# j042/mimi

Measured on AMD Instinct MI355X. Metric: element-integrations/sec (residual+Jacobian assembly), higher is better.
Workload: dtype f64

## Files before the change

mimi_amd/csrc/kernels_tensor_wgs.hpp:

```cpp
#pragma once

#include <hip/hip_runtime.h>

#include "materials_other.hpp"

#include "kernels_tensor_2phase.hpp"

namespace mimi_hip {

struct P2Shape {
  static constexpr int P = 2, NB = 3, NQ = 4, NB2 = 9, ND = 27, NQ3 = 64, NROW = 81;
};

constexpr int p2_stage_r_size(int rows) {
  using S = P2Shape;
  return rows * 3 * (S::NQ3 + S::NB * S::NQ * S::NQ + S::NB2 * S::NQ);
}

struct WgsLds : P2Shape {
  static constexpr int off_tab = 0;
  static constexpr int off_r = off_tab + 2 * 6 * NB * NQ;
  static constexpr int off_ah = off_r + p2_stage_r_size(1);
  static constexpr int n_final = 9 * NROW + 18 * ND;
  static constexpr int n_carry = 18 * 2 * ND;
  static constexpr int st_size = n_final + 1;
  static constexpr int off_st = off_ah + 3 * ND * NQ3;
  static constexpr int total = off_st + 3 * st_size;
};

#define WGS_PIN(x) asm volatile("" : "+v"(x))

MH_DEV void wgs_barrier() {
  asm volatile("s_waitcnt lgkmcnt(0)\n\ts_barrier" ::: "memory");
}

MH_DEV void swap32_f64(double c, double o, double& c_hi_in_lo, double& o_lo_in_hi) {
  const unsigned long long uc = __double_as_longlong(c), uo = __double_as_longlong(o);
  const auto lo = __builtin_amdgcn_permlane32_swap((unsigned)uc, (unsigned)uo, false, false);
  const auto hi = __builtin_amdgcn_permlane32_swap((unsigned)(uc >> 32), (unsigned)(uo >> 32), false, false);
  o_lo_in_hi = __longlong_as_double(((unsigned long long)hi[0] << 32) | lo[0]);
  c_hi_in_lo = __longlong_as_double(((unsigned long long)hi[1] << 32) | lo[1]);
}

constexpr int WGS_PT_FIELDS = 24;

MH_DEV void wgs_point_store(double* rec, int lane, const mimi_hip_material& m, const PointResult<3>& w) {
  constexpr int NQ3 = P2Shape::NQ3;
  constexpr int sym_i[6] = {0, 1, 2, 1, 2, 2}, sym_j[6] = {0, 0, 0, 1, 1, 2};
#pragma unroll
  for (int k = 0; k < 9; ++k) rec[k * NQ3 + lane] = w.Finv[k];
  rec[9 * NQ3 + lane] = w.detF;
#pragma unroll
  for (int k = 0; k < 6; ++k) {
    rec[(10 + k) * NQ3 + lane] = w.sigma[sym_i[k] + 3 * sym_j[k]];
    rec[(16 + k) * NQ3 + lane] = w.s_trial[sym_i[k] + 3 * sym_j[k]];
  }
  double beta, gamma;
  j2_beta_gamma<3>(m, w, beta, gamma);
  rec[22 * NQ3 + lane] = beta;
  rec[23 * NQ3 + lane] = gamma;
}

MH_DEV void wgs_point_load(const double* rec, int lane, PointResult<3>& w, double& beta, double& gamma) {
  constexpr int NQ3 = P2Shape::NQ3;
  constexpr int sym_i[6] = {0, 1, 2, 1, 2, 2}, sym_j[6] = {0, 0, 0, 1, 1, 2};
#pragma unroll
  for (int k = 0; k < 9; ++k) w.Finv[k] = rec[k * NQ3 + lane];
  w.detF = rec[9 * NQ3 + lane];
#pragma unroll
  for (int k = 0; k < 6; ++k) {
    const double sg = rec[(10 + k) * NQ3 + lane], st = rec[(16 + k) * NQ3 + lane];
    w.sigma[sym_i[k] + 3 * sym_j[k]] = sg;
    w.sigma[sym_j[k] + 3 * sym_i[k]] = sg;
    w.s_trial[sym_i[k] + 3 * sym_j[k]] = st;
    w.s_trial[sym_j[k] + 3 * sym_i[k]] = st;
  }
  beta = rec[22 * NQ3 + lane];
  gamma = rec[23 * NQ3 + lane];
  pk1_from_cauchy<3>(w);
}

constexpr int WGS_REC_FIELDS = 90;
constexpr int WGS_KIND_RECORD = 100;

template<int FAMILY, int COMMIT = 0>
__global__ __launch_bounds__(256) void tensor_point_kernel(TensorArgs p, int n_el) {
  constexpr int P = P2Shape::P, NB = P2Shape::NB, NQ = P2Shape::NQ, ND = P2Shape::ND, NQ3 = P2Shape::NQ3;
  constexpr int FK = family_kind<FAMILY>();
  __shared__ double ue_all[4][3 * ND];
  __shared__ double tab_all[4][6 * NB * NQ];
  const int wave = threadIdx.x >> 6, lane = threadIdx.x & 63;
  const int64_t e = (int64_t)blockIdx.x * 4 + wave;
  if (e >= n_el) return;
  double* ue = ue_all[wave];
  double* tab = tab_all[wave];
  int el[3];
  el[0] = e % p.box_n[0];
  el[1] = (e / p.box_n[0]) % p.box_n[1];
  el[2] = e / ((int64_t)p.box_n[0] * p.box_n[1]);
  const int32_t* dofs = p.dofs + e * ND;
  for (int a = lane; a < ND; a += 64) {
    const int64_t node = dofs[a];
    for (int c = 0; c < 3; ++c) ue[c * ND + a] = p.u[node * 3 + c];
  }
  for (int t = lane; t < 6 * NB * NQ; t += 64) {
    const int dir = t / (2 * NB * NQ), rem = t % (2 * NB * NQ), isD = rem / (NB * NQ), k = rem % (NB * NQ);
    const int span = p.box_begin[dir] + el[dir];
    tab[t] = ((isD ? p.tabD[dir] : p.tabB[dir]) + (int64_t)span * NB * NQ)[k];
  }
  __builtin_amdgcn_s_waitcnt(0);
  __builtin_amdgcn_wave_barrier();
  const int q0 = lane % NQ, q1 = (lane / NQ) % NQ, q2 = lane / (NQ * NQ);
  double H[9];
  for (int k = 0; k < 9; ++k) H[k] = 0.0;
#pragma unroll 1
  for (int a2 = 0; a2 < NB; ++a2)
#pragma unroll 1
    for (int a1 = 0; a1 < NB; ++a1)
      for (int a0 = 0; a0 < NB; ++a0) {
        const int a = a0 + NB * (a1 + NB * a2);
        const double b0 = tab_ptr<P>(tab, 0, 0)[a0 * NQ + q0], d0 = tab_ptr<P>(tab, 0, 1)[a0 * NQ + q0];
        const double b1 = tab_ptr<P>(tab, 1, 0)[a1 * NQ + q1], d1 = tab_ptr<P>(tab, 1, 1)[a1 * NQ + q1];
        const double b2 = tab_ptr<P>(tab, 2, 0)[a2 * NQ + q2], d2 = tab_ptr<P>(tab, 2, 1)[a2 * NQ + q2];
        const double dn0 = d0 * (b1 * b2), dn1 = b0 * (d1 * b2), dn2 = b0 * (b1 * d2);
        for (int i = 0; i < 3; ++i) {
          const double uu = ue[i * ND + a];
          H[i * 3 + 0] += uu * dn0;
          H[i * 3 + 1] += uu * dn1;
          H[i * 3 + 2] += uu * dn2;
        }
      }
  const double* g = p.geo + e * 10 * NQ3 + lane;
  double F[9];
  for (int i = 0; i < 3; ++i)
    for (int J = 0; J < 3; ++J) {
      double sf = (i == J) ? 1.0 : 0.0;
      for (int m = 0; m < 3; ++m) sf += H[i * 3 + m] * g[(int64_t)(m * 3 + J) * NQ3];
      F[i + J * 3] = sf;
    }
  if constexpr (COMMIT) {
    int st;
    if constexpr (FAMILY != 0) st = accumulate_other<3, FK>(p.mat, p.dt, p.state, e * NQ3 + lane, F);
    else st = accumulate_state<3>(p.mat, p.dt, p.state, e * NQ3 + lane, F);
    if (st) atomicOr(p.status, st);
    return;
  }
  if constexpr (FAMILY != 0) {
    double Pk[9];
    OtherTangent<3> ot;
    const int status = other_tangent_begin<3, FK>(p.mat, p.dt, p.state, e * NQ3 + lane, F, Pk, ot);
    double* rec = p.scratch_pt + e * (int64_t)(WGS_REC_FIELDS * NQ3) + lane;
    const double wd = g[(int64_t)9 * NQ3];
    double Ji[9];
#pragma unroll
    for (int k = 0; k < 9; ++k) Ji[k] = g[(int64_t)k * NQ3];
#pragma unroll 1
    for (int j = 0; j < 3; ++j) {
      double acc[27];
#pragma unroll
      for (int k = 0; k < 27; ++k) acc[k] = 0.0;
#pragma unroll 1
      for (int L = 0; L < 3; ++L) {
        double dP[9];
        other_tangent_dir<3, FK>(p.mat, p.dt, F, ot, j, L, dP);
        double jl[3];
#pragma unroll
        for (int n = 0; n < 3; ++n) jl[n] = L == 0 ? Ji[n * 3] : (L == 1 ? Ji[n * 3 + 1] : Ji[n * 3 + 2]);
#pragma unroll
        for (int i = 0; i < 3; ++i)
#pragma unroll
          for (int m = 0; m < 3; ++m) {
            double b = 0.0;
#pragma unroll
            for (int J = 0; J < 3; ++J) b += Ji[m * 3 + J] * dP[i + J * 3];
#pragma unroll
            for (int n = 0; n < 3; ++n) acc[(i * 3 + m) * 3 + n] += b * jl[n];
          }
      }
#pragma unroll
      for (int i = 0; i < 3; ++i)
#pragma unroll
        for (int m = 0; m < 3; ++m)
#pragma unroll
          for (int n = 0; n < 3; ++n) rec[(int64_t)(i * 27 + (m * 3 + j) * 3 + n) * NQ3] = wd * acc[(i * 3 + m) * 3 + n];
    }
#pragma unroll
    for (int i = 0; i < 3; ++i)
#pragma unroll
      for (int m = 0; m < 3; ++m) {
        double t = 0.0;
#pragma unroll
        for (int J = 0; J < 3; ++J) t += Pk[i + J * 3] * Ji[m * 3 + J];
        rec[(int64_t)(81 + i * 3 + m) * NQ3] = wd * t;
      }
    if (status) atomicOr(p.status, status);
  } else {
    PointResult<3> w;
    const int status = evaluate_pk1<3>(p.mat, p.dt, p.state, e * NQ3 + lane, F, w);
    wgs_point_store(p.scratch_pt + e * (int64_t)(WGS_PT_FIELDS * NQ3), lane, p.mat.m, w);
    if (status) atomicOr(p.status, status);
  }
}

template<int KIND>
struct WgsPoint;

template<>
struct WgsPoint<MIMI_HIP_MAT_NEOHOOKEAN> {
  double G[9], M[6], Phat[9];
  double mu_w, c1_w, c2_w;
};

template<>
struct WgsPoint<MIMI_HIP_MAT_J2> {
  double G[9], Ji[9], N[9], Q[9], sig[9], st[9], Phat[9];
  double wdJ, Kc, hb, gg;
};

template<>
struct WgsPoint<WGS_KIND_RECORD> {
  const double* rec;
};

MH_DEV void wgs_j2_point(const mimi_hip_material& m, const PointResult<3>& w, double beta, double gamma, const double* Ji,
                         double wd, WgsPoint<MIMI_HIP_MAT_J2>& s) {
  const double G2 = 2.0 * m.G;
  s.wdJ = wd * w.detF;
  s.Kc = m.K - beta * G2 / 3.0;
  s.hb = 0.5 * beta * G2;
  s.gg = G2 * gamma;
#pragma unroll
  for (int k = 0; k < 9; ++k) {
    s.Ji[k] = Ji[k];
    s.sig[k] = w.sigma[k];
    s.st[k] = w.s_trial[k];
  }
#pragma unroll
  for (int mm = 0; mm < 3; ++mm)
#pragma unroll
    for (int c = 0; c < 3; ++c) {
      double g = 0.0;
#pragma unroll
      for (int Jx = 0; Jx < 3; ++Jx) g += Ji[mm * 3 + Jx] * w.Finv[Jx + c * 3];
      s.G[mm * 3 + c] = g;
    }
#pragma unroll
  for (int mm = 0; mm < 3; ++mm)
#pragma unroll
    for (int n = 0; n < 3; ++n) {
      double v = 0.0;
#pragma unroll
      for (int k = 0; k < 3; ++k) v += s.G[mm * 3 + k] * Ji[n * 3 + k];
      s.N[mm * 3 + n] = v;
    }
#pragma unroll
  for (int n = 0; n < 3; ++n)
#pragma unroll
    for (int j = 0; j < 3; ++j) {
      double v = 0.0;
#pragma unroll
      for (int Lx = 0; Lx < 3; ++Lx) v += w.s_trial[j + Lx * 3] * Ji[n * 3 + Lx];
      s.Q[n * 3 + j] = v;
    }
#pragma unroll
  for (int i = 0; i < 3; ++i)
#pragma unroll
    for (int mm = 0; mm < 3; ++mm) {
      double sp = 0.0;
#pragma unroll
      for (int Jx = 0; Jx < 3; ++Jx) sp += w.P[i + Jx * 3] * Ji[mm * 3 + Jx];
      s.Phat[i * 3 + mm] = wd * sp;
    }
}

MH_DEV void wgs_neohookean_point(const mimi_hip_material& mat, const double* F, const double* Ji, double wd,
                                 WgsPoint<MIMI_HIP_MAT_NEOHOOKEAN>& s) {
  PointResult<3> w;
  neo_hookean_stress<3>(mat, F, w);
  const double J = w.detF;
  s.mu_w = wd * mat.mu;
  s.c1_w = wd * (mat.lambda * J * (J - 1.) - mat.mu);
  s.c2_w = wd * (mat.lambda * (2. * J - 1.) * J);
#pragma unroll
  for (int m = 0; m < 3; ++m)
#pragma unroll
    for (int i = 0; i < 3; ++i) {
      double g = 0.0;
#pragma unroll
      for (int Jx = 0; Jx < 3; ++Jx) g += Ji[m * 3 + Jx] * w.Finv[Jx + i * 3];
      s.G[m * 3 + i] = g;
    }
  {
    int c = 0;
#pragma unroll
    for (int m = 0; m < 3; ++m)
#pragma unroll
      for (int n = m; n < 3; ++n) {
        double v = 0.0;
#pragma unroll
        for (int Jx = 0; Jx < 3; ++Jx) v += Ji[m * 3 + Jx] * Ji[n * 3 + Jx];
        s.M[c++] = v;
      }
  }
#pragma unroll
  for (int i = 0; i < 3; ++i)
#pragma unroll
    for (int m = 0; m < 3; ++m) {
      double sp = 0.0;
#pragma unroll
      for (int Jx = 0; Jx < 3; ++Jx) sp += w.P[i + Jx * 3] * Ji[m * 3 + Jx];
      s.Phat[i * 3 + m] = wd * sp;
    }
}

template<int ROWS>
MH_DEV void p2_stage_r(const double* tab, double* RS, int lane, double* er, int I0) {
  using S = P2Shape;
  constexpr int P = S::P, NB = S::NB, NQ = S::NQ, NB2 = S::NB2, ND = S::ND, NQ3 = S::NQ3;
  double* PH = RS;
  double* V = PH + ROWS * 3 * NQ3;
  double* W = V + ROWS * 3 * NB * NQ * NQ;
  __builtin_amdgcn_wave_barrier();
  if (lane < NB * NQ * NQ) {
    const int q01 = lane & 15, a2 = lane >> 4;
    double T[2][NQ];
#pragma unroll
    for (int v = 0; v < 2; ++v)
#pragma unroll
      for (int q2 = 0; q2 < NQ; ++q2) T[v][q2] = tab_ptr<P>(tab, 2, v)[a2 * NQ + q2];
#pragma unroll
    for (int im = 0; im < ROWS * 3; ++im) {
      double sv = 0.0;
#pragma unroll
      for (int q2 = 0; q2 < NQ; ++q2) sv = __builtin_fma(T[im % 3 == 2 ? 1 : 0][q2], PH[im * NQ3 + q01 + NQ * NQ * q2], sv);
      V[im * (NB * NQ * NQ) + lane] = sv;
    }
  }
  __builtin_amdgcn_wave_barrier();
  if (lane < NB2 * NQ) {
    const int q0 = lane & 3, a12 = lane >> 2, a1 = a12 % NB, a2 = a12 / NB;
    double T[2][NQ];
#pragma unroll
    for (int v = 0; v < 2; ++v)
#pragma unroll
      for (int q1 = 0; q1 < NQ; ++q1) T[v][q1] = tab_ptr<P>(tab, 1, v)[a1 * NQ + q1];
#pragma unroll
    for (int im = 0; im < ROWS * 3; ++im) {
      double sw = 0.0;
#pragma unroll
      for (int q1 = 0; q1 < NQ; ++q1) sw = __builtin_fma(T[im % 3 == 1 ? 1 : 0][q1], V[(im * NB + a2) * NQ * NQ + q0 + NQ * q1], sw);
      W[im * (NB2 * NQ) + lane] = sw;
    }
  }
  __builtin_amdgcn_wave_barrier();
  if (lane < (ROWS > 1 ? 2 : 1) * ND) {
    const int a = lane < ND ? lane : lane - ND, a0 = a % NB, a12 = a / NB;
    double T[2][NQ];
#pragma unroll
    for (int v = 0; v < 2; ++v)
#pragma unroll
      for (int q0 = 0; q0 < NQ; ++q0) T[v][q0] = tab_ptr<P>(tab, 0, v)[a0 * NQ + q0];
    const int n_rows = lane < ND ? (ROWS + 1) / 2 : ROWS / 2;
    for (int k = 0; k < n_rows; ++k) {
      const int I = lane < ND ? 2 * k : 2 * k + 1;
      double sr = 0.0;
#pragma unroll
      for (int m = 0; m < 3; ++m)
#pragma unroll
        for (int q0 = 0; q0 < NQ; ++q0) sr = __builtin_fma(T[m == 0 ? 1 : 0][q0], W[((I * 3 + m) * NB2 + a12) * NQ + q0], sr);
      er[a * 3 + I0 + I] = sr;
    }
  }
  __builtin_amdgcn_wave_barrier();
}

template<int KIND, int I>
MH_DEV void wgs_x_row(const TensorArgs& p, double* lds, int lane, int64_t e, int par, const WgsPoint<KIND>& s) {
  using L = WgsLds;
  constexpr int NB = L::NB, NQ = L::NQ, ND = L::ND, NQ3 = L::NQ3;
  static_assert(KIND == MIMI_HIP_MAT_J2 || KIND == WGS_KIND_RECORD, "nine-block kernel: the material comes from the pre-pass");
  const double* tab = lds + L::off_tab + par * 6 * NB * NQ;
  double* AH = lds + L::off_ah + I * ND * NQ3;
  double* RS = lds + L::off_r;
  double Phat[3];
  if constexpr (KIND == WGS_KIND_RECORD) {
#pragma unroll
    for (int m = 0; m < 3; ++m) Phat[m] = s.rec[(int64_t)(81 + I * 3 + m) * NQ3];
    double v[ND];
#pragma unroll
    for (int k = 0; k < ND; ++k) v[k] = s.rec[(int64_t)(I * ND + k) * NQ3];
#pragma unroll
    for (int k = 0; k < ND; ++k) AH[k * NQ3 + lane] = v[k];
  } else {
#pragma unroll
    for (int m = 0; m < 3; ++m) Phat[m] = s.Phat[I * 3 + m];
    double S[3], Ts[3];
#pragma unroll
    for (int m = 0; m < 3; ++m) {
      double a = 0.0, b = 0.0;
#pragma unroll
      for (int k = 0; k < 3; ++k) {
        a += s.sig[I + k * 3] * s.G[m * 3 + k];
        b += s.st[I + k * 3] * s.G[m * 3 + k];
      }
      S[m] = a;
      Ts[m] = b;
    }
#pragma unroll
    for (int m = 0; m < 3; ++m)
#pragma unroll
      for (int j = 0; j < 3; ++j)
#pragma unroll
        for (int n = 0; n < 3; ++n) {
          double v = s.G[n * 3 + j] * S[m] - s.G[m * 3 + j] * S[n];
          v += s.Kc * s.G[m * 3 + I] * s.Ji[n * 3 + j];
          v += s.hb * ((I == j ? s.N[m * 3 + n] : 0.0) + s.G[m * 3 + j] * s.Ji[n * 3 + I]);
          v -= s.gg * Ts[m] * s.Q[n * 3 + j];
          AH[((m * 3 + j) * 3 + n) * NQ3 + lane] = s.wdJ * v;
        }
  }
#pragma unroll
  for (int m = 0; m < 3; ++m) RS[m * NQ3 + lane] = Phat[m];
  p2_stage_r<1>(tab, RS, lane, p.scratch_r + e * ND * 3, I);
}

struct ColumnWalk {
  int first, nseg;
  int g, pos, unit;
  int cx, cy, ez;
  int64_t e;
  MH_DEV ColumnWalk(const TensorArgs& p, int first_unit) : first(first_unit), nseg(p.box_n[2] / p.seg_len), g(0) { begin_unit(p, 0); }
  MH_DEV void begin_unit(const TensorArgs& p, int u) {
    const int un = first + u, col = un / nseg;
    unit = u;
    pos = 0;
    cx = col % p.box_n[0];
    cy = col / p.box_n[0];
    ez = (un % nseg) * p.seg_len;
    e = cx + (int64_t)p.box_n[0] * (cy + (int64_t)p.box_n[1] * ez);
  }
  MH_DEV void advance(const TensorArgs& p) {
    ++g;
    if (++pos == p.seg_len) {
      begin_unit(p, unit + 1);
    } else {
      ++ez;
      e += (int64_t)p.box_n[0] * p.box_n[1];
    }
  }
};

struct WgsOperands {
  static constexpr int NT = 6 * P2Shape::NB * P2Shape::NQ, TROUNDS = 2;
  double tab[TROUNDS], geo[10];
  MH_DEV static const double* table_src(const TensorArgs& p, const ColumnWalk& c, int t) {
    constexpr int NBQ = P2Shape::NB * P2Shape::NQ;
    const int dir = t / (2 * NBQ);
    const int rem = t % (2 * NBQ);
    const int isD = rem / NBQ;
    const int k = rem % NBQ;
    const int span = (dir == 0 ? p.box_begin[0] + c.cx : dir == 1 ? p.box_begin[1] + c.cy : p.box_begin[2] + c.ez);
    return (isD ? (dir == 0 ? p.tabD[0] : dir == 1 ? p.tabD[1] : p.tabD[2])
                : (dir == 0 ? p.tabB[0] : dir == 1 ? p.tabB[1] : p.tabB[2])) + (int64_t)span * NBQ + k;
  }
  MH_DEV void request(const TensorArgs& p, const ColumnWalk& c, int lane) {
#pragma unroll
    for (int rd = 0; rd < TROUNDS; ++rd) {
      const int t = rd * 64 + lane;
      tab[rd] = *table_src(p, c, t < NT ? t : 0);
    }
    const double* g = p.geo + c.e * 10 * P2Shape::NQ3 + lane;
#pragma unroll
    for (int k = 0; k < 10; ++k) geo[k] = g[(int64_t)k * P2Shape::NQ3];
  }
  MH_DEV void tables_to_lds(double* dst, int lane) const {
#pragma unroll
    for (int rd = 0; rd < TROUNDS; ++rd) {
      const int t = rd * 64 + lane;
      if (t < NT) dst[t] = tab[rd];
    }
  }
};

template<int KIND>
MH_DEV void wgs_x_loop(const TensorArgs& p, double* lds, int unit) {
  using L = WgsLds;
  const int lane = threadIdx.x & 63;
  const int n_seq = p.seg_len;
  ColumnWalk cq(p, unit);
  ColumnWalk cs = cq;
  ColumnWalk cr = cq;
  WgsOperands op;
  auto request = [&]() {
    op.request(p, cq, lane);
    if (cq.g + 1 < n_seq) cq.advance(p);
  };
  WgsPoint<KIND> s;
  auto point_stage = [&]() {
    op.tables_to_lds(lds + L::off_tab + (cs.g & 1) * WgsOperands::NT, lane);
    if constexpr (KIND == WGS_KIND_RECORD) {
      s.rec = p.scratch_pt + cs.e * (int64_t)(WGS_REC_FIELDS * L::NQ3) + lane;
    } else {
      PointResult<3> w;
      double beta, gamma;
      wgs_point_load(p.scratch_pt + cs.e * (int64_t)(WGS_PT_FIELDS * L::NQ3), lane, w, beta, gamma);
      wgs_j2_point(p.mat.m, w, beta, gamma, op.geo, op.geo[9], s);
    }
    __builtin_amdgcn_wave_barrier();
    if (cs.g + 1 < n_seq) cs.advance(p);
  };
  auto rows = [&]() {
    wgs_x_row<KIND, 0>(p, lds, lane, cr.e, cr.g & 1, s);
    wgs_x_row<KIND, 1>(p, lds, lane, cr.e, cr.g & 1, s);
    wgs_x_row<KIND, 2>(p, lds, lane, cr.e, cr.g & 1, s);
  };
  request();
  point_stage();
  if (1 < n_seq) request();
  rows();
  wgs_barrier();
  for (int it = 0; it < n_seq; ++it) {
    if (it + 1 < n_seq) {
      point_stage();
      if (it + 2 < n_seq) request();
    }
    wgs_barrier();
    if (it + 1 < n_seq) {
      cr.advance(p);
      rows();
    }
    wgs_barrier();
  }
}

struct WgsLane {
  int lane, grp;
  bool col_ok;
  double take_c0, take_c1;
  int base0, stride0, base1, basec;
  int baseT0, strideT0, baseT1, basecT;
};

MH_DEV WgsLane wgs_lane_constants(bool for_dump = false) {
  constexpr int NB = P2Shape::NB, ND = P2Shape::ND, NROW = P2Shape::NROW;
  WgsLane c;
  c.lane = threadIdx.x & 63;
  const int col = c.lane & 15;
  c.grp = c.lane >> 4;
  c.col_ok = col < 9;
  c.take_c0 = c.grp != 2 ? 1.0 : 0.0;
  c.take_c1 = c.grp == 0 ? 1.0 : 0.0;
  const int a0 = c.col_ok ? col / NB : 0, b0 = c.col_ok ? col % NB : 0;
  const int grp = c.grp;
  c.base0 = grp < 3 ? a0 * NROW + grp * ND + b0 * 3 : 9 * NROW + a0 * ND + b0 * 3;
  c.stride0 = grp < 3 ? 3 * NROW : 3 * ND;
  c.base1 = 9 * NROW + (a0 + 9) * ND + b0 * 3;
  c.basec = a0 * 162 + b0 * 3 + (grp == 0 ? 0 : grp == 1 ? ND : grp == 3 ? 9 * 162 : 9 * 162 + ND);
  c.baseT0 = grp == 0 ? b0 * NROW + a0 * 3
           : grp == 3 ? b0 * NROW + ND + a0 * 3
           : grp == 1 ? 9 * NROW + b0 * ND + a0 * 3
                      : 9 * NROW + (b0 + 9) * ND + a0 * 3;
  c.strideT0 = (grp == 0 || grp == 3) ? 3 * NROW : 3 * ND;
  c.baseT1 = b0 * NROW + 2 * ND + a0 * 3;
  c.basecT = b0 * 162 + a0 * 3 + (grp == 0 ? 0 : grp == 1 ? 9 * 162 : grp == 3 ? ND : 9 * 162 + ND);
  if (for_dump) {
    if (!c.col_ok) c.base0 = c.stride0 = c.baseT0 = c.strideT0 = 0;
    if (!c.col_ok || grp != 2) c.base1 = c.baseT1 = 0;
  }
  return c;
}

template<int MODE, bool DUMP = false>
MH_DEV void wgs_contract_block(const WgsLane& lc, const double (&ah)[9], const double (&aS0)[4], const double (&aS2)[4],
                               const double (&uB1)[3][4], const double (&uD1)[3][4], double (&C)[9],
                               double* st_n, int jn, double* st_t, int jt, double* dump = nullptr) {
  constexpr int NB = P2Shape::NB, NQ = P2Shape::NQ, ND = P2Shape::ND, NROW = P2Shape::NROW;
  const mh_d4 zero4 = {0.0, 0.0, 0.0, 0.0};
  const int grp = lc.grp;
  double* const dn0 = lc.col_ok ? st_n : dump;
  double* const dn1 = (lc.col_ok && grp == 2) ? st_n : dump;
  double* const dt0 = lc.col_ok ? st_t : dump;
  double* const dt1 = (lc.col_ok && grp == 2) ? st_t : dump;
  mh_d4 D1[9];
#pragma unroll
  for (int mn = 0; mn < 9; ++mn) {
    const int m = mn / 3, n = mn % 3;
    const int v2 = (m == 2 ? 1 : 0) + (n == 2 ? 2 : 0);
    if (MODE == 2 && mn == 3) D1[3] = D1[1];
    else D1[mn] = __builtin_amdgcn_mfma_f64_16x16x4f64(ah[mn], aS2[v2], zero4, 0, 0, 0);
  }
  mh_d4 Kt[NB];
  auto carry_and_stage = [&](int b1) {
#pragma unroll
    for (int a1 = 0; a1 < NB; ++a1) {
      if (MODE == 2 && a1 < b1) continue;
      const int a1b1 = a1 * NB + b1;
      const double cin = C[a1b1];
      double c_rot, o2_rot;
      swap32_f64(cin, Kt[a1][2], c_rot, o2_rot);
      const double out0 = MODE == 0 ? Kt[a1][0] + (grp != 2 ? cin : 0.0) : __builtin_fma(cin, lc.take_c0, Kt[a1][0]);
      const double out1 = MODE == 0 ? Kt[a1][1] + (grp == 0 ? c_rot : 0.0) : __builtin_fma(c_rot, lc.take_c1, Kt[a1][1]);
      if constexpr (DUMP) {
        dn0[lc.base0 + a1 * lc.stride0 + b1 * 9 + jn] = out0;
        dn1[lc.base1 + a1 * (3 * ND) + b1 * 9 + jn] = out1;
        if (MODE == 1 || (MODE == 2 && a1 > b1)) {
          dt0[lc.baseT0 + b1 * lc.strideT0 + a1 * 9 + jt] = out0;
          dt1[lc.baseT1 + b1 * (3 * NROW) + a1 * 9 + jt] = out1;
        }
      } else {
        if (lc.col_ok) st_n[lc.base0 + a1 * lc.stride0 + b1 * 9 + jn] = out0;
        if (lc.col_ok && grp == 2) st_n[lc.base1 + a1 * (3 * ND) + b1 * 9 + jn] = out1;
        if (MODE == 1 || (MODE == 2 && a1 > b1)) {
          if (lc.col_ok) st_t[lc.baseT0 + b1 * lc.strideT0 + a1 * 9 + jt] = out0;
          if (lc.col_ok && grp == 2) st_t[lc.baseT1 + b1 * (3 * NROW) + a1 * 9 + jt] = out1;
        }
      }
      C[a1b1] = grp == 2 ? o2_rot : out1;
    }
  };
#pragma unroll
  for (int b1 = 0; b1 < NB; ++b1) {
    double Ec[4][NB];
#pragma unroll
    for (int q1 = 0; q1 < NQ; ++q1) {
      const double cbB = uB1[b1][q1], cbD = uD1[b1][q1];
      const double W3 = cbB * D1[0][q1];
      const double W1 = __builtin_fma(cbD, D1[1][q1], cbB * D1[2][q1]);
      const double W2a = cbB * D1[3][q1], W2b = cbB * D1[6][q1];
      const double W0a = __builtin_fma(cbD, D1[4][q1], cbB * D1[5][q1]);
      const double W0b = __builtin_fma(cbD, D1[7][q1], cbB * D1[8][q1]);
#pragma unroll
      for (int a1 = 0; a1 < NB; ++a1) {
        if (MODE == 2 && a1 < b1) continue;
        const double caB = uB1[a1][q1], caD = uD1[a1][q1];
        if (q1 == 0) {
          Ec[3][a1] = caB * W3;
          Ec[1][a1] = caB * W1;
          Ec[2][a1] = __builtin_fma(caD, W2a, caB * W2b);
          Ec[0][a1] = __builtin_fma(caD, W0a, caB * W0b);
        } else {
          Ec[3][a1] = __builtin_fma(caB, W3, Ec[3][a1]);
          Ec[1][a1] = __builtin_fma(caB, W1, Ec[1][a1]);
          Ec[2][a1] = __builtin_fma(caD, W2a, __builtin_fma(caB, W2b, Ec[2][a1]));
          Ec[0][a1] = __builtin_fma(caD, W0a, __builtin_fma(caB, W0b, Ec[0][a1]));
        }
      }
    }
    if (b1 > 0) carry_and_stage(b1 - 1);
#pragma unroll
    for (int g = 0; g < 4; ++g)
#pragma unroll
      for (int a1 = 0; a1 < NB; ++a1)
        if (!(MODE == 2 && a1 < b1)) WGS_PIN(Ec[g][a1]);
#pragma unroll
    for (int a1 = 0; a1 < NB; ++a1)
      if (!(MODE == 2 && a1 < b1)) Kt[a1] = __builtin_amdgcn_mfma_f64_16x16x4f64(Ec[0][a1], aS0[0], zero4, 0, 0, 0);
#pragma unroll
    for (int g = 1; g < 4; ++g)
#pragma unroll
      for (int a1 = 0; a1 < NB; ++a1)
        if (!(MODE == 2 && a1 < b1)) Kt[a1] = __builtin_amdgcn_mfma_f64_16x16x4f64(Ec[g][a1], aS0[g], Kt[a1], 0, 0, 0);
  }
  carry_and_stage(NB - 1);
}

template<int MODE>
MH_DEV void wgs_stage_carry(const WgsLane& lc, const double (&C)[9], double* st_n, int jn, double* st_t, int jt) {
  constexpr int NB = P2Shape::NB;
#pragma unroll
  for (int a1b1 = 0; a1b1 < 9; ++a1b1) {
    const int a1 = a1b1 / NB, b1 = a1b1 % NB;
    if (MODE == 2 && a1 < b1) continue;
    if (lc.col_ok) st_n[lc.basec + a1 * 486 + b1 * 9 + jn] = C[a1b1];
    if ((MODE == 1 || (MODE == 2 && a1 > b1)) && lc.col_ok) st_t[lc.basecT + b1 * 486 + a1 * 9 + jt] = C[a1b1];
  }
}

#define WGS_PIECE_STORE(ptr, v) (*(ptr) = (v))
MH_DEV void wgs_flush_final(int lane, const double* ST, double* E, int I) {
  constexpr int NROW = P2Shape::NROW, ND = P2Shape::ND;
  {
    const int g3 = lane / 17, k3 = lane - 17 * g3;
    const bool ok3 = lane < 51;
    const int src3 = ok3 ? g3 * NROW + 64 + k3 : 0, dst3 = g3 * 3 * NROW + 64 + k3;
    double v0[9], v1[3];
#pragma unroll
    for (int a = 0; a < 9; ++a) v0[a] = ST[a * NROW + lane];
#pragma unroll
    for (int q = 0; q < 3; ++q) v1[q] = ST[q * 3 * NROW + src3];
    double* d = E + I * NROW;
#pragma unroll
    for (int a = 0; a < 9; ++a) WGS_PIECE_STORE(&d[(unsigned)(a * 3 * NROW + lane)], v0[a]);
#pragma unroll
    for (int q = 0; q < 3; ++q)
      if (ok3) WGS_PIECE_STORE(&d[(unsigned)(q * 9 * NROW + dst3)], v1[q]);
  }
  {
    const int half = lane >> 5, k = lane & 31;
    const bool ok = k < ND;
    double w[9];
#pragma unroll
    for (int r = 0; r < 9; ++r) w[r] = ST[9 * NROW + (2 * r + half) * ND + (ok ? k : 0)];
    double* d = E + P2Block::off_b20 + I * ND + half * NROW + k;
#pragma unroll
    for (int r = 0; r < 9; ++r)
      if (ok) WGS_PIECE_STORE(&d[(unsigned)(2 * r * NROW)], w[r]);
  }
}

MH_DEV void wgs_load_tables(const double* tab, int lane, bool column_too, double (&aS0)[4], double (&aS2)[4],
                            double (&uB1)[P2Shape::NB][P2Shape::NQ], double (&uD1)[P2Shape::NB][P2Shape::NQ]) {
  constexpr int P = P2Shape::P, NB = P2Shape::NB, NQ = P2Shape::NQ;
  const int mrow = lane & 15, mk = lane >> 4;
  const bool mrow_ok = mrow < P2Shape::NB2;
  const int mra = mrow_ok ? mrow / NB : 0, mrb = mrow_ok ? mrow % NB : 0;
  auto pair_products = [&](int dir, double (&aS)[4]) {
    const double Ba = tab_ptr<P>(tab, dir, 0)[mra * NQ + mk], Da = tab_ptr<P>(tab, dir, 1)[mra * NQ + mk];
    const double Bb = tab_ptr<P>(tab, dir, 0)[mrb * NQ + mk], Db = tab_ptr<P>(tab, dir, 1)[mrb * NQ + mk];
    aS[0] = mrow_ok ? Ba * Bb : 0.0;
    aS[1] = mrow_ok ? Da * Bb : 0.0;
    aS[2] = mrow_ok ? Ba * Db : 0.0;
    aS[3] = mrow_ok ? Da * Db : 0.0;
  };
  if (column_too) {
    pair_products(0, aS0);
#pragma unroll
    for (int a = 0; a < NB; ++a)
#pragma unroll
      for (int q1 = 0; q1 < NQ; ++q1) {
        const unsigned long long vb = __double_as_longlong(tab_ptr<P>(tab, 1, 0)[a * NQ + q1]);
        const unsigned long long vd = __double_as_longlong(tab_ptr<P>(tab, 1, 1)[a * NQ + q1]);
        const unsigned blo = __builtin_amdgcn_readfirstlane((unsigned)vb), bhi = __builtin_amdgcn_readfirstlane((unsigned)(vb >> 32));
        const unsigned dlo = __builtin_amdgcn_readfirstlane((unsigned)vd), dhi = __builtin_amdgcn_readfirstlane((unsigned)(vd >> 32));
        uB1[a][q1] = __longlong_as_double(((unsigned long long)bhi << 32) | blo);
        uD1[a][q1] = __longlong_as_double(((unsigned long long)dhi << 32) | dlo);
      }
  }
  pair_products(2, aS2);
}

template<int I>
MH_DEV void wgs_y_loop(const TensorArgs& p, double* lds, int unit) {
  using L = WgsLds;
  constexpr int NB = L::NB, NQ = L::NQ, NB2 = L::NB2, ND = L::ND, NQ3 = L::NQ3;
  const WgsLane lc = wgs_lane_constants();
  const int lane = lc.lane;
  double* AH = lds + L::off_ah + I * ND * NQ3;
  double* ST = lds + L::off_st + I * L::st_size;
  const int n_seq = p.seg_len;
  ColumnWalk c(p, unit);
  auto block_of = [&](int64_t e) -> double* { return p.scratch_k + e * (int64_t)P2Block::size; };

  double C[3][NB2];
#pragma unroll
  for (int j = 0; j < 3; ++j)
#pragma unroll
    for (int k = 0; k < NB2; ++k) C[j][k] = 0.0;
  double aS0[4], aS2[4];
  double uB1[NB][NQ], uD1[NB][NQ];
  auto load_slice = [&](int j, double (&ah)[9]) {
#pragma unroll
    for (int m = 0; m < 3; ++m)
#pragma unroll
      for (int n = 0; n < 3; ++n) ah[m * 3 + n] = AH[((m * 3 + j) * 3 + n) * NQ3 + lane];
  };
  wgs_barrier();
  for (int it = 0; it < n_seq; ++it) {
    wgs_load_tables(lds + L::off_tab + (it & 1) * WgsOperands::NT, lane, true, aS0, aS2, uB1, uD1);
    {
      double ah[9];
      load_slice(0, ah);
      wgs_contract_block<0>(lc, ah, aS0, aS2, uB1, uD1, C[0], ST, 0, ST, 0);
    }
    {
      double ah[9];
      load_slice(1, ah);
      wgs_contract_block<0>(lc, ah, aS0, aS2, uB1, uD1, C[1], ST, 1, ST, 1);
    }
    {
      double ah[9];
      load_slice(2, ah);
      wgs_barrier();
      wgs_contract_block<0>(lc, ah, aS0, aS2, uB1, uD1, C[2], ST, 2, ST, 2);
      __builtin_amdgcn_wave_barrier();
      wgs_flush_final(lane, ST, block_of(c.e), I);
      __builtin_amdgcn_wave_barrier();
      wgs_barrier();
    }
    if (it + 1 < n_seq) c.advance(p);
  }
  {
    double* Sc = P2Block::carry_of(block_of(c.e), I);
#pragma unroll
    for (int jj = 0; jj < 3; ++jj) wgs_stage_carry<0>(lc, C[jj], Sc, jj, Sc, jj);
  }
}

template<int KIND>
__global__ __launch_bounds__(256, 2) void tensor_wgs_kernel(TensorArgs p) {
  extern __shared__ __align__(16) double smem_wgs[];
#ifndef WGS_ROT
#define WGS_ROT(b) ((b) >> 3)
#endif
  const int role = __builtin_amdgcn_readfirstlane((int)((threadIdx.x >> 6) + WGS_ROT(blockIdx.x)) & 3);
  const int unit = blockIdx.x;
  if (role == 0) wgs_x_loop<KIND>(p, smem_wgs, unit);
  else if (role == 1) wgs_y_loop<0>(p, smem_wgs, unit);
  else if (role == 2) wgs_y_loop<1>(p, smem_wgs, unit);
  else wgs_y_loop<2>(p, smem_wgs, unit);
}

inline void launch_tensor_wgs(mimi_hip_domain_s* h, const DomainCall& c, TensorArgs a) {
  h->scratch_k.resize((size_t)h->n_el * P2Block::size);
  h->scratch_r.resize((size_t)h->n_el * 3 * 27);
  a.scratch_k = h->scratch_k.ptr;
  a.scratch_r = h->scratch_r.ptr;
  a.n_units_u = a.box_n[0];
  a.n_units_v = a.box_n[1];
  const size_t lds = WgsLds::total * sizeof(double);
  const int kind = h->mat.m.kind;
  h->scratch_pt.resize((size_t)h->n_el * (material_closed_form(kind) ? WGS_PT_FIELDS : WGS_REC_FIELDS) * 64);
  a.scratch_pt = h->scratch_pt.ptr;
  by_material_family(kind, [&](auto K) {
    constexpr int FK = decltype(K)::value;
    run_two_phase(
        h, c, true,
        [&] { launch(tensor_point_kernel<FK>, dim3((unsigned)((h->n_el + 3) / 4)), dim3(256), 0, h->stream, a, (int)h->n_el); },
        [&] {
          auto kernel = FK != 0 ? tensor_wgs_kernel<WGS_KIND_RECORD> : tensor_wgs_kernel<MIMI_HIP_MAT_J2>;
          launch(kernel, dim3(a.box_n[0] * a.box_n[1]), dim3(256), lds, h->stream, a);
        },
        [&] { launch_tensor_p2(h, a); });
  });
}

inline void launch_tensor_p2_post(mimi_hip_domain_s* h, TensorArgs a) {
  by_material_family(h->mat.m.kind, [&](auto K) {
    launch(tensor_point_kernel<decltype(K)::value, 1>, dim3((unsigned)((h->n_el + 3) / 4)), dim3(256), 0, h->stream, a, (int)h->n_el);
  });
}

}
```

mimi_amd/csrc/kernels_tensor_wgsym.hpp:

```cpp
#pragma once

#include <hip/hip_runtime.h>

#include "kernels_tensor_wgs.hpp"

namespace mimi_hip {

#ifndef WGSYM_SPLIT_BELOW
#define WGSYM_SPLIT_BELOW 512
#endif
#ifndef WGSYM_MAX_COLS
#define WGSYM_MAX_COLS 4
#define WGSYM_MIN_WGS 2048
#endif

#ifndef WGSYM_DIAG_MODE
#define WGSYM_DIAG_MODE 2
#endif

struct WgsymLds : P2Shape {
  static constexpr int off_ue = 0;
  static constexpr int off_tab = off_ue + 3 * ND + 1;
  static constexpr int off_r = off_tab + 2 * 6 * NB * NQ;
  static constexpr int off_ah = off_r + p2_stage_r_size(3);
  static constexpr int off_st = off_ah + 6 * 9 * NQ3;
  static constexpr int off_dump = off_st + 3 * WgsLds::st_size;
  static constexpr int total = off_dump + 512;
  MH_DEV static constexpr int ah_block(int i, int j) { return (i * (i + 1) / 2 + j) * 9; }
};

template<int KIND>
MH_DEV void wgsym_x_rows(const TensorArgs& p, double* lds, int lane, int64_t e, int par, const WgsPoint<KIND>& s) {
  using L = WgsymLds;
  constexpr int ND = L::ND, NQ3 = L::NQ3;
  static_assert(KIND == MIMI_HIP_MAT_NEOHOOKEAN, "symmetric-half kernel: hyperelastic materials only");
  const double* tab = lds + L::off_tab + par * WgsOperands::NT;
  double* AH = lds + L::off_ah;
  double* PH = lds + L::off_r;
#pragma unroll
  for (int I = 0; I < 3; ++I)
#pragma unroll
    for (int m = 0; m < 3; ++m) {
      const double c2gm = s.c2_w * s.G[m * 3 + I];
#pragma unroll
      for (int j = 0; j <= I; ++j) {
        const double c1gm = s.c1_w * s.G[m * 3 + j];
#pragma unroll
        for (int n = 0; n < 3; ++n) {
          double v = c2gm * s.G[n * 3 + j] - c1gm * s.G[n * 3 + I];
          if (I == j) {
            const int lo = m < n ? m : n, hi = m < n ? n : m;
            v += s.mu_w * s.M[lo * 3 - lo * (lo - 1) / 2 + (hi - lo)];
          }
          AH[(L::ah_block(I, j) + m * 3 + n) * NQ3 + lane] = v;
        }
      }
    }
#pragma unroll
  for (int k = 0; k < 9; ++k) PH[k * NQ3 + lane] = s.Phat[k];
  p2_stage_r<3>(tab, PH, lane, p.scratch_r + e * ND * 3, 0);
}

template<int KIND>
MH_DEV void wgsym_x_loop(const TensorArgs& p, double* lds, int col0, int n_cols) {
  using L = WgsymLds;
  constexpr int P = L::P, NB = L::NB, NQ = L::NQ, ND = L::ND;
  const int lane = threadIdx.x & 63;
  double* ue = lds + L::off_ue;
  const int n_seq = n_cols * p.seg_len;
  ColumnWalk cq(p, col0);
  ColumnWalk cs = cq;
  ColumnWalk cr = cq;
  int32_t node_n = lane < ND ? p.dofs[cq.e * ND + lane] : 0;
  double ue_r[3];
  WgsOperands op;
  auto request = [&]() {
#pragma unroll
    for (int c = 0; c < 3; ++c) ue_r[c] = p.u[(int64_t)node_n * 3 + c];
    op.request(p, cq, lane);
    if (cq.g + 1 < n_seq) {
      cq.advance(p);
      node_n = lane < ND ? p.dofs[cq.e * ND + lane] : 0;
    }
  };
  WgsPoint<KIND> s;
  auto point_stage = [&]() {
    double* tab = lds + L::off_tab + (cs.g & 1) * WgsOperands::NT;
    if (lane < ND) {
#pragma unroll
      for (int c = 0; c < 3; ++c) ue[c * ND + lane] = ue_r[c];
    }
    op.tables_to_lds(tab, lane);
    double Ji[9];
#pragma unroll
    for (int k = 0; k < 9; ++k) Ji[k] = op.geo[k];
    const double wd = op.geo[9];
    __builtin_amdgcn_wave_barrier();
    double F[9];
    {
      const int q0 = lane & 3, q1 = (lane >> 2) & 3, q2 = lane >> 4;
      double b0[NB], d0[NB], b1[NB], d1[NB], b2[NB], d2[NB];
#pragma unroll
      for (int a = 0; a < NB; ++a) {
        b0[a] = tab_ptr<P>(tab, 0, 0)[a * NQ + q0];
        d0[a] = tab_ptr<P>(tab, 0, 1)[a * NQ + q0];
        b1[a] = tab_ptr<P>(tab, 1, 0)[a * NQ + q1];
        d1[a] = tab_ptr<P>(tab, 1, 1)[a * NQ + q1];
        b2[a] = tab_ptr<P>(tab, 2, 0)[a * NQ + q2];
        d2[a] = tab_ptr<P>(tab, 2, 1)[a * NQ + q2];
      }
      double H[9];
#pragma unroll
      for (int k = 0; k < 9; ++k) H[k] = 0.0;
#pragma unroll
      for (int a2 = 0; a2 < NB; ++a2)
#pragma unroll
        for (int a1 = 0; a1 < NB; ++a1) {
          const double tbb = b1[a1] * b2[a2], tdb = d1[a1] * b2[a2], tbd = b1[a1] * d2[a2];
#pragma unroll
          for (int a0 = 0; a0 < NB; ++a0) {
            const int a = a0 + NB * (a1 + NB * a2);
            const double dn0 = d0[a0] * tbb, dn1 = b0[a0] * tdb, dn2 = b0[a0] * tbd;
#pragma unroll
            for (int i = 0; i < 3; ++i) {
              const double uu = ue[i * ND + a];
              H[i * 3 + 0] += uu * dn0;
              H[i * 3 + 1] += uu * dn1;
              H[i * 3 + 2] += uu * dn2;
            }
          }
          #pragma unroll
          for (int k = 0; k < 9; ++k) asm volatile("" : "+v"(H[k]) : : "memory");
        }
#pragma unroll
      for (int i = 0; i < 3; ++i)
#pragma unroll
        for (int J = 0; J < 3; ++J) {
          double sf = (i == J) ? 1.0 : 0.0;
#pragma unroll
          for (int m = 0; m < 3; ++m) sf += H[i * 3 + m] * Ji[m * 3 + J];
          F[i + J * 3] = sf;
        }
    }
    wgs_neohookean_point(p.mat.m, F, Ji, wd, s);
    __builtin_amdgcn_wave_barrier();
    if (cs.g + 1 < n_seq) cs.advance(p);
  };

  request();
  point_stage();
  if (1 < n_seq) request();
  wgsym_x_rows<KIND>(p, lds, lane, cr.e, 0, s);
  wgs_barrier();
  for (int it = 0; it < n_seq; ++it) {
    if (it + 1 < n_seq) {
      point_stage();
      if (it + 2 < n_seq) request();
    }
    wgs_barrier();
    if (it + 1 < n_seq) {
      cr.advance(p);
      wgsym_x_rows<KIND>(p, lds, lane, cr.e, (it + 1) & 1, s);
    }
    wgs_barrier();
  }
}

template<int W>
MH_DEV void wgsym_y_loop(const TensorArgs& p, double* lds, int col0, int n_cols) {
  using L = WgsymLds;
  constexpr int NB2 = L::NB2, NQ3 = L::NQ3;
  constexpr int I1 = W == 0 ? 1 : 2, J1 = W == 2 ? 1 : 0;
  const WgsLane lc = wgs_lane_constants(true);
  const int lane = lc.lane;
  const int n_seq = n_cols * p.seg_len;
  const double* AH0 = lds + L::off_ah + L::ah_block(W, W) * NQ3;
  const double* AH1 = lds + L::off_ah + L::ah_block(I1, J1) * NQ3;
  auto st_of = [&](int piece) -> double* { return lds + L::off_st + piece * WgsLds::st_size; };
  auto block_at = [&](int64_t e) -> double* { return p.scratch_k + e * (int64_t)P2Block::size; };
  ColumnWalk c(p, col0);
  int64_t e_prev = c.e;

  double C0[NB2], C1[NB2];
#pragma unroll
  for (int k = 0; k < NB2; ++k) C0[k] = C1[k] = 0.0;
  double aS0[4], aS2[4];
  double uB1[L::NB][L::NQ], uD1[L::NB][L::NQ];

  wgs_barrier();
  for (int it = 0; it < n_seq; ++it) {
    {
      if (it >= 1) wgs_flush_final(lane, st_of(W), block_at(e_prev), W);
      wgs_load_tables(lds + L::off_tab + (it & 1) * WgsOperands::NT, lane, c.pos == 0, aS0, aS2, uB1, uD1);
      double ah[9];
#pragma unroll
      for (int k = 0; k < 9; ++k) ah[k] = AH0[k * NQ3 + lane];
      wgs_contract_block<WGSYM_DIAG_MODE, true>(lc, ah, aS0, aS2, uB1, uD1, C0, st_of(W), W, st_of(W), W, lds + L::off_dump);
    }
    {
      double ah[9];
#pragma unroll
      for (int k = 0; k < 9; ++k) ah[k] = AH1[k * NQ3 + lane];
      wgs_barrier();
      wgs_contract_block<1, true>(lc, ah, aS0, aS2, uB1, uD1, C1, st_of(I1), J1, st_of(J1), I1, lds + L::off_dump);
      wgs_barrier();
      if (c.pos == p.seg_len - 1) {
        double* E = block_at(c.e);
        wgs_stage_carry<WGSYM_DIAG_MODE>(lc, C0, P2Block::carry_of(E, W), W, P2Block::carry_of(E, W), W);
        wgs_stage_carry<1>(lc, C1, P2Block::carry_of(E, I1), J1, P2Block::carry_of(E, J1), I1);
#pragma unroll
        for (int k = 0; k < NB2; ++k) C0[k] = C1[k] = 0.0;
      }
    }
    e_prev = c.e;
    if (it + 1 < n_seq) c.advance(p);
  }
  wgs_flush_final(lane, st_of(W), block_at(e_prev), W);
}

template<int KIND>
__global__ __launch_bounds__(256, 2) void tensor_wgsym_kernel(TensorArgs p) {
  extern __shared__ __align__(16) double smem_wgsym[];
  const int role = __builtin_amdgcn_readfirstlane((int)((threadIdx.x >> 6) + WGS_ROT(blockIdx.x)) & 3);
  const int n_cols_all = p.box_n[0] * p.box_n[1] * (p.box_n[2] / p.seg_len);
  const int col0 = blockIdx.x * p.cols_per_wg;
  const int n_cols = n_cols_all - col0 < p.cols_per_wg ? n_cols_all - col0 : p.cols_per_wg;
  if (role == 0) wgsym_x_loop<KIND>(p, smem_wgsym, col0, n_cols);
  else if (role == 1) wgsym_y_loop<0>(p, smem_wgsym, col0, n_cols);
  else if (role == 2) wgsym_y_loop<1>(p, smem_wgsym, col0, n_cols);
  else wgsym_y_loop<2>(p, smem_wgsym, col0, n_cols);
}

inline void launch_tensor_wgsym(mimi_hip_domain_s* h, const DomainCall& c, TensorArgs a) {
  h->scratch_k.resize((size_t)h->n_el * P2Block::size);
  h->scratch_r.resize((size_t)h->n_el * 3 * 27);
  a.scratch_k = h->scratch_k.ptr;
  a.scratch_r = h->scratch_r.ptr;
  a.n_units_u = a.box_n[0];
  a.n_units_v = a.box_n[1];
  const size_t lds = WgsymLds::total * sizeof(double);
  int nseg = 1;
  while (a.box_n[0] * a.box_n[1] * nseg * 2 <= WGSYM_SPLIT_BELOW && a.box_n[2] % (nseg * 2) == 0 && a.box_n[2] / (nseg * 2) >= 4) nseg *= 2;
  a.seg_len = a.box_n[2] / nseg;
  const int n_cols_all = a.box_n[0] * a.box_n[1] * nseg;
  a.cols_per_wg = n_cols_all / WGSYM_MIN_WGS < 1 ? 1 : (n_cols_all / WGSYM_MIN_WGS > WGSYM_MAX_COLS ? WGSYM_MAX_COLS : n_cols_all / WGSYM_MIN_WGS);
  run_two_phase(
      h, c, false, [] {},
      [&] {
        launch(tensor_wgsym_kernel<MIMI_HIP_MAT_NEOHOOKEAN>, dim3((n_cols_all + a.cols_per_wg - 1) / a.cols_per_wg), dim3(256), lds,
               h->stream, a);
      },
      [&] { launch_tensor_p2(h, a); });
}

}
```

Baseline: 37.47 million.

## Pack rider a1 tile rows into neighboring MFMA tiles to skip one MFMA chain

For off-diagonal blocks (MODE 1, b1<2), the rows of the a1=1 tile are shifted via DPP row moves into unused rows of the a1=0 and a1=2 MFMA tiles. This removes one 4-MFMA chain per packed b1 step. The carry for the packed tile moves into a new LDS region (CP), which adds LDS traffic and remapped store addresses, and the LDS budget is asserted against two workgroups per CU. It also adds DPP cross-lane operations and more complex indexing, which could offset the MFMA savings.

```diff
diff --git a/mimi_amd/csrc/kernels_tensor_wgs.hpp b/mimi_amd/csrc/kernels_tensor_wgs.hpp
--- a/mimi_amd/csrc/kernels_tensor_wgs.hpp
+++ b/mimi_amd/csrc/kernels_tensor_wgs.hpp
@@ -5,6 +5,7 @@
 #include "materials_other.hpp"
 
 #include "kernels_tensor_2phase.hpp"
+#include "p2_tile_map.hpp"
 
 namespace mimi_hip {
 
@@ -570,11 +571,45 @@
   return c;
 }
 
-template<int MODE, bool DUMP = false>
+struct WgsPackLane {
+  bool ok2, ok3;
+  bool take2, wide2;
+  int base2, baseT2;
+  int base3, baseT3;
+};
+
+MH_DEV WgsPackLane wgs_pack_lane_constants(const WgsLane& lc) {
+  constexpr int ND = P2Shape::ND, NROW = P2Shape::NROW, NB = P2Shape::NB;
+  WgsPackLane c;
+  const int col = lc.lane & 15, grp = lc.grp;
+  const int a0 = lc.col_ok ? col / NB : 0, b0 = lc.col_ok ? col % NB : 0;
+  c.ok2 = lc.col_ok && grp >= 1;
+  c.ok3 = lc.col_ok && (grp == 0 || grp == 3);
+  c.take2 = grp == 1 || grp == 2;
+  c.wide2 = grp == 1;
+  c.base2 = c.ok2 ? a0 * NROW + (grp - 1) * ND + b0 * 3 : 0;
+  c.baseT2 = !c.ok2 ? 0 : grp == 1 ? b0 * NROW + a0 * 3 : 9 * NROW + (b0 + 9 * (grp - 2)) * ND + a0 * 3;
+  c.base3 = c.ok3 ? 9 * NROW + (a0 + (grp == 3 ? 9 : 0)) * ND + b0 * 3 : 0;
+  c.baseT3 = c.ok3 ? b0 * NROW + (grp == 3 ? 2 : 1) * ND + a0 * 3 : 0;
+  return c;
+}
+
+template<int N, int BANKS>
+MH_DEV double wgs_rows_up(double dst, double src) {
+  const unsigned long long ud = __double_as_longlong(dst), us = __double_as_longlong(src);
+  const unsigned lo = (unsigned)__builtin_amdgcn_update_dpp((int)(unsigned)ud, (int)(unsigned)us, 0x110 + N, 0xf, BANKS, false);
+  const unsigned hi = (unsigned)__builtin_amdgcn_update_dpp((int)(unsigned)(ud >> 32), (int)(unsigned)(us >> 32), 0x110 + N, 0xf, BANKS, false);
+  return __longlong_as_double(((unsigned long long)hi << 32) | lo);
+}
+
+template<int MODE, bool DUMP = false, int PACK = 0>
 MH_DEV void wgs_contract_block(const WgsLane& lc, const double (&ah)[9], const double (&aS0)[4], const double (&aS2)[4],
                                const double (&uB1)[3][4], const double (&uD1)[3][4], double (&C)[9],
-                               double* st_n, int jn, double* st_t, int jt, double* dump = nullptr) {
+                               double* st_n, int jn, double* st_t, int jt, double* dump = nullptr,
+                               const WgsPackLane* pl = nullptr, double* CP = nullptr) {
   constexpr int NB = P2Shape::NB, NQ = P2Shape::NQ, ND = P2Shape::ND, NROW = P2Shape::NROW;
+  static_assert(!PACK || (DUMP && MODE != 0), "packed tiles: symmetric-half kernel only");
+  static_assert(P2_RIDER == 1 && p2_tile_slot(0, 8).tile == 0 && p2_tile_slot(2, 8).tile == 1, "hosts a1 = 0, 2");
   const mh_d4 zero4 = {0.0, 0.0, 0.0, 0.0};
   const int grp = lc.grp;
   double* const dn0 = lc.col_ok ? st_n : dump;
@@ -591,9 +626,28 @@
   }
   mh_d4 Kt[NB];
   auto carry_and_stage = [&](int b1) {
+    const bool packed = p2_b1_packed(MODE, b1, PACK);
+    if (packed) {
+      constexpr int a1 = P2_RIDER;
+      double* const d2n = pl->ok2 ? st_n : dump;
+      double* const d3n = pl->ok3 ? st_n : dump;
+      double* const d2t = pl->ok2 ? st_t : dump;
+      double* const d3t = pl->ok3 ? st_t : dump;
+      const double out3 = __builtin_fma(CP[b1 * 64 + lc.lane], 1.0, Kt[0][3]);
+      const double out2 = __builtin_fma(pl->take2 ? C[a1 * NB + b1] : 0.0, 1.0, Kt[0][2]);
+      d2n[pl->base2 + a1 * (3 * NROW) + b1 * 9 + jn] = out2;
+      d3n[pl->base3 + a1 * (3 * ND) + b1 * 9 + jn] = out3;
+      if (MODE == 1 || (MODE == 2 && a1 > b1)) {
+        d2t[pl->baseT2 + (pl->wide2 ? b1 * (3 * NROW) : b1 * (3 * ND)) + a1 * 9 + jt] = out2;
+        d3t[pl->baseT3 + b1 * (3 * NROW) + a1 * 9 + jt] = out3;
+      }
+      C[a1 * NB + b1] = out3;
+      CP[b1 * 64 + lc.lane] = Kt[2][3];
+    }
 #pragma unroll
     for (int a1 = 0; a1 < NB; ++a1) {
       if (MODE == 2 && a1 < b1) continue;
+      if (packed && a1 == P2_RIDER) continue;
       const int a1b1 = a1 * NB + b1;
       const double cin = C[a1b1];
       double c_rot, o2_rot;
@@ -652,25 +706,56 @@
 #pragma unroll
       for (int a1 = 0; a1 < NB; ++a1)
         if (!(MODE == 2 && a1 < b1)) WGS_PIN(Ec[g][a1]);
+    const bool packed = p2_b1_packed(MODE, b1, PACK);
+    if (packed) {
+      static_assert(p2_tile_slot(P2_RIDER, 0).row == P2_RIDER_SHIFT_LOW && p2_tile_slot(P2_RIDER, 8).row == 8 + P2_RIDER_SHIFT_HIGH);
+#pragma unroll
+      for (int g = 0; g < 4; ++g) {
+        Ec[g][0] = wgs_rows_up<P2_RIDER_SHIFT_LOW, 0xf>(Ec[g][0], Ec[g][P2_RIDER]);
+        Ec[g][2] = wgs_rows_up<P2_RIDER_SHIFT_HIGH, 0x8>(Ec[g][2], Ec[g][P2_RIDER]);
+      }
+#pragma unroll
+      for (int g = 0; g < 4; ++g) {
+        WGS_PIN(Ec[g][0]);
+        WGS_PIN(Ec[g][2]);
+      }
+    }
 #pragma unroll
     for (int a1 = 0; a1 < NB; ++a1)
-      if (!(MODE == 2 && a1 < b1)) Kt[a1] = __builtin_amdgcn_mfma_f64_16x16x4f64(Ec[0][a1], aS0[0], zero4, 0, 0, 0);
+      if (!(MODE == 2 && a1 < b1) && !(packed && a1 == P2_RIDER)) Kt[a1] = __builtin_amdgcn_mfma_f64_16x16x4f64(Ec[0][a1], aS0[0], zero4, 0, 0, 0);
 #pragma unroll
     for (int g = 1; g < 4; ++g)
 #pragma unroll
       for (int a1 = 0; a1 < NB; ++a1)
-        if (!(MODE == 2 && a1 < b1)) Kt[a1] = __builtin_amdgcn_mfma_f64_16x16x4f64(Ec[g][a1], aS0[g], Kt[a1], 0, 0, 0);
+        if (!(MODE == 2 && a1 < b1) && !(packed && a1 == P2_RIDER)) Kt[a1] = __builtin_amdgcn_mfma_f64_16x16x4f64(Ec[g][a1], aS0[g], Kt[a1], 0, 0, 0);
   }
   carry_and_stage(NB - 1);
 }
 
-template<int MODE>
-MH_DEV void wgs_stage_carry(const WgsLane& lc, const double (&C)[9], double* st_n, int jn, double* st_t, int jt) {
-  constexpr int NB = P2Shape::NB;
+template<int MODE, int PACK = 0>
+MH_DEV void wgs_stage_carry(const WgsLane& lc, const double (&C)[9], double* st_n, int jn, double* st_t, int jt,
+                            const double* CP = nullptr) {
+  constexpr int NB = P2Shape::NB, ND = P2Shape::ND;
 #pragma unroll
   for (int a1b1 = 0; a1b1 < 9; ++a1b1) {
     const int a1 = a1b1 / NB, b1 = a1b1 % NB;
     if (MODE == 2 && a1 < b1) continue;
+    if (p2_b1_packed(MODE, b1, PACK) && a1 == P2_RIDER) {
+      const int col = lc.lane & 15, grp = lc.grp;
+      const int a0 = lc.col_ok ? col / NB : 0, b0 = lc.col_ok ? col % NB : 0;
+      const int n0 = a0 * 162 + b0 * 3 + a1 * 486 + b1 * 9 + jn, t0 = b0 * 162 + a0 * 3 + b1 * 486 + a1 * 9 + jt;
+      const bool tr = MODE == 1 || (MODE == 2 && a1 > b1);
+      if (lc.col_ok && (grp == 1 || grp == 2)) {
+        st_n[n0 + (grp == 2 ? ND : 0)] = C[a1b1];
+        if (tr) st_t[t0 + (grp == 2 ? 9 * 162 : 0)] = C[a1b1];
+      }
+      if (lc.col_ok && grp < 2) {
+        const double cp = CP[b1 * 64 + lc.lane];
+        st_n[n0 + 9 * 162 + (grp == 1 ? ND : 0)] = cp;
+        if (tr) st_t[t0 + ND + (grp == 1 ? 9 * 162 : 0)] = cp;
+      }
+      continue;
+    }
     if (lc.col_ok) st_n[lc.basec + a1 * 486 + b1 * 9 + jn] = C[a1b1];
     if ((MODE == 1 || (MODE == 2 && a1 > b1)) && lc.col_ok) st_t[lc.basecT + b1 * 486 + a1 * 9 + jt] = C[a1b1];
   }
diff --git a/mimi_amd/csrc/kernels_tensor_wgsym.hpp b/mimi_amd/csrc/kernels_tensor_wgsym.hpp
--- a/mimi_amd/csrc/kernels_tensor_wgsym.hpp
+++ b/mimi_amd/csrc/kernels_tensor_wgsym.hpp
@@ -12,6 +12,10 @@
 #ifndef WGSYM_MAX_COLS
 #define WGSYM_MAX_COLS 4
 #define WGSYM_MIN_WGS 2048
+#endif
+
+#ifndef WGSYM_PACK
+#define WGSYM_PACK 1
 #endif
 
 #ifndef WGSYM_DIAG_MODE
@@ -25,7 +29,9 @@
   static constexpr int off_ah = off_r + p2_stage_r_size(3);
   static constexpr int off_st = off_ah + 6 * 9 * NQ3;
   static constexpr int off_dump = off_st + 3 * WgsLds::st_size;
-  static constexpr int total = off_dump + 512;
+  static constexpr int off_cp = off_dump + 512;
+  static constexpr int total = off_cp + 3 * 4 * 64;
+  static_assert(2 * total * sizeof(double) <= 160 * 1024, "two workgroups per CU");
   MH_DEV static constexpr int ah_block(int i, int j) { return (i * (i + 1) / 2 + j) * 9; }
 };
 
@@ -172,6 +178,7 @@
   constexpr int NB2 = L::NB2, NQ3 = L::NQ3;
   constexpr int I1 = W == 0 ? 1 : 2, J1 = W == 2 ? 1 : 0;
   const WgsLane lc = wgs_lane_constants(true);
+  const WgsPackLane pl = wgs_pack_lane_constants(lc);
   const int lane = lc.lane;
   const int n_seq = n_cols * p.seg_len;
   const double* AH0 = lds + L::off_ah + L::ah_block(W, W) * NQ3;
@@ -184,6 +191,10 @@
   double C0[NB2], C1[NB2];
 #pragma unroll
   for (int k = 0; k < NB2; ++k) C0[k] = C1[k] = 0.0;
+  double* const CP0 = lds + L::off_cp + W * 4 * 64;
+  double* const CP1 = CP0 + 64;
+#pragma unroll
+  for (int k = 0; k < 4; ++k) CP0[k * 64 + lane] = 0.0;
   double aS0[4], aS2[4];
   double uB1[L::NB][L::NQ], uD1[L::NB][L::NQ];
 
@@ -195,21 +206,24 @@
       double ah[9];
 #pragma unroll
       for (int k = 0; k < 9; ++k) ah[k] = AH0[k * NQ3 + lane];
-      wgs_contract_block<WGSYM_DIAG_MODE, true>(lc, ah, aS0, aS2, uB1, uD1, C0, st_of(W), W, st_of(W), W, lds + L::off_dump);
+      wgs_contract_block<WGSYM_DIAG_MODE, true, WGSYM_PACK>(lc, ah, aS0, aS2, uB1, uD1, C0, st_of(W), W, st_of(W), W, lds + L::off_dump,
+                                                                   &pl, CP0);
     }
     {
       double ah[9];
 #pragma unroll
       for (int k = 0; k < 9; ++k) ah[k] = AH1[k * NQ3 + lane];
       wgs_barrier();
-      wgs_contract_block<1, true>(lc, ah, aS0, aS2, uB1, uD1, C1, st_of(I1), J1, st_of(J1), I1, lds + L::off_dump);
+      wgs_contract_block<1, true, WGSYM_PACK>(lc, ah, aS0, aS2, uB1, uD1, C1, st_of(I1), J1, st_of(J1), I1, lds + L::off_dump, &pl, CP1);
       wgs_barrier();
       if (c.pos == p.seg_len - 1) {
         double* E = block_at(c.e);
-        wgs_stage_carry<WGSYM_DIAG_MODE>(lc, C0, P2Block::carry_of(E, W), W, P2Block::carry_of(E, W), W);
-        wgs_stage_carry<1>(lc, C1, P2Block::carry_of(E, I1), J1, P2Block::carry_of(E, J1), I1);
+        wgs_stage_carry<WGSYM_DIAG_MODE, WGSYM_PACK>(lc, C0, P2Block::carry_of(E, W), W, P2Block::carry_of(E, W), W, CP0);
+        wgs_stage_carry<1, WGSYM_PACK>(lc, C1, P2Block::carry_of(E, I1), J1, P2Block::carry_of(E, J1), I1, CP1);
 #pragma unroll
         for (int k = 0; k < NB2; ++k) C0[k] = C1[k] = 0.0;
+#pragma unroll
+        for (int k = 0; k < 4; ++k) CP0[k * 64 + lane] = 0.0;
       }
     }
     e_prev = c.e;
diff --git a/mimi_amd/csrc/p2_tile_map.hpp b/mimi_amd/csrc/p2_tile_map.hpp
--- /dev/null
+++ b/mimi_amd/csrc/p2_tile_map.hpp
@@ -0,0 +1,26 @@
+#pragma once
+
+namespace mimi_hip {
+
+struct P2TileSlot {
+  int tile, row;
+};
+
+constexpr int P2_TILES_PACKED = 2;
+constexpr int P2_RIDER = 1;
+constexpr int P2_RIDER_SPLIT = 7;
+constexpr int P2_RIDER_SHIFT_LOW = 9;
+constexpr int P2_RIDER_SHIFT_HIGH = 5;
+
+constexpr P2TileSlot p2_tile_slot(int a1, int pair) {
+  return a1 == 0   ? P2TileSlot{0, pair}
+         : a1 == 2 ? P2TileSlot{1, pair}
+         : pair < P2_RIDER_SPLIT ? P2TileSlot{0, pair + P2_RIDER_SHIFT_LOW}
+                                 : P2TileSlot{1, pair + P2_RIDER_SHIFT_HIGH};
+}
+
+constexpr bool p2_b1_packed(int mode, int b1, int level) {
+  return level >= 2 ? mode == 1 || (mode == 2 && b1 == 0) : level == 1 && mode == 1 && b1 < 2;
+}
+
+}
```

Result: faster. 38.69 million, median of 6 (+3.3%).
